# multiplefish/VPLines-SLAM

Hardware: AMD Instinct MI355X
Metric: sliding-window BA solves/sec (10 KF, 200 pts + 80 lines, 5 iters) (higher is better)
Workload: dtype f64

## Files before the change

include/vplines_ba.h:

```cpp
#ifndef VPLINES_BA_H
#define VPLINES_BA_H

#ifdef __cplusplus
extern "C" {
#endif

#define VPL_WINDOW_SIZE 10
#define VPL_NFRAMES 11
#define VPL_MAX_PRIOR_BLOCKS 23
#define VPL_MAX_PRIOR_DIM 171

#define VPL_OK 0
#define VPL_E_INVALID -1
#define VPL_E_NODEVICE -2
#define VPL_E_HIP -3
#define VPL_E_CAPACITY -4
#define VPL_E_NUMERIC -5

#define VPL_MARGIN_OLD 0
#define VPL_MARGIN_SECOND_NEW 1
#define VPL_MARGIN_NONE -1

#define VPL_BLOCK_POSE 0
#define VPL_BLOCK_SPEEDBIAS 1
// ... 266 lines not shown
int vpl_odo_solve_auto(vpl_odo* odo, vpl_odo_result* out);
int vpl_odo_keyframe_auto(vpl_odo* odo, const vpl_odo_frame* next, vpl_odo_result* out);
int vpl_odo_keyframe_imu_auto(vpl_odo* odo, const vpl_odo_imu_frame* next, vpl_odo_result* out, vpl_odo_imu_out* imu_out);

int vpl_odo_get_prior(vpl_odo* odo, int seq, vpl_prior* out);
int vpl_odo_get_states(vpl_odo* odo, int seq, double (*pose)[7], double (*speed_bias)[9], double* ex_pose);
int vpl_odo_get_tracks(vpl_odo* odo, int seq, int* n_points, int* point_id, int* point_start, int* point_nobs, double* inv_depth,
                       int* n_lines, int* line_id, int* line_start, int* line_nobs, int* line_triangulated, double* line_plk);
#define VPL_ODO_D2H_PAD_BYTES 0
int vpl_odo_stats(vpl_odo* odo, long long* h2d_payload_bytes, long long* h2d_table_bytes, long long* d2h_bytes);
int vpl_odo_debug_ms(vpl_odo* odo, double* ms4);

int vpl_odo_debug_tracks(int max_tracks, int n_steps, const int* flag, const int* n_ids, const int* ids, const unsigned char* erase,
                         int* status, int* n_slide, int* slide, int* n_tracks, int* table, int* ignored);
int vpl_odo_debug_parallax_list(int max_tracks, int n_steps, const int* flag, const int* n_ids, const int* ids,
                                const unsigned char* erase, int* n_list, int* list, int* last_track_num);

int vpl_ba_debug_linearization(vpl_ctx* ctx, int window, int* n_points, int* n_lines, int* line_index, double* H, double* g,
                               double* x_pose, double* x_speed_bias, double* x_ex_pose, double* x_inv_depth, double* x_line_orth,
                               double* x_cost);
int vpl_ba_debug_step(vpl_ctx* ctx, int window, double* scale, double* diag, double* grad, double* gn, double* tr14, int* path,
                      double* cand_pose, double* cand_speed_bias, double* cand_ex_pose, double* cand_inv_depth,
                      double* cand_line_orth);

int vpl_ba_enable_kernel_timing(vpl_ctx* ctx, int enable);
int vpl_ba_kernel_times(vpl_ctx* ctx, int* count, const char** names, double* total_ms, int* launches);
int vpl_ba_launch_profile(vpl_ctx* ctx, int* count, const char** names, double* ms, int* active);

int vpl_ba_debug_point_units(int n_points, const int* point_start, const int* point_nobs, int max_rounds,
                             int* lane_table, int* unit_table, int* rounds, int* rounds0);
int vpl_ba_debug_point_chains(const int* unit_table, int rounds, int rounds0, int marg_pass);

#ifdef __cplusplus
}
#endif
#endif
```

vplines-slam_amd/capi.py:

```python
import ctypes as C
import time
import os

import numpy as np

from . import _build

NF = 11
MAX_PRIOR_BLOCKS = 23
MAX_PRIOR_DIM = 171
MARGIN_OLD, MARGIN_SECOND_NEW, MARGIN_NONE = 0, 1, -1
PRIOR_PIVOTED_CHOLESKY, PRIOR_EIGEN = 0, 1
BLOCK_POSE, BLOCK_SPEEDBIAS, BLOCK_EXPOSE = 0, 1, 2

_dp = C.POINTER(C.c_double)
_ip = C.POINTER(C.c_int)


class BaOptions(C.Structure):
    _fields_ = [("num_iterations", C.c_int), ("estimate_extrinsic", C.c_int), ("marginalization_flag", C.c_int),
                ("remove_line_outliers", C.c_int), ("focal_length", C.c_double), ("line_factor", C.c_double),
                ("vp_factor", C.c_double), ("g_norm", C.c_double), ("acc_n", C.c_double), ("gyr_n", C.c_double),
                ("acc_w", C.c_double), ("gyr_w", C.c_double), ("huber_delta", C.c_double)]

# ... 319 lines not shown
    lib.vpl_odo_enable_imu.argtypes = [vp, C.c_int]
    lib.vpl_odo_set_imu.argtypes = [vp, C.c_int, C.c_int, _dp, _dp, _dp]
    lib.vpl_odo_advance_imu.argtypes = [vp, C.POINTER(OdoImuFrame), C.POINTER(OdoResult), C.POINTER(OdoImuOut)]
    lib.vpl_odo_keyframe_imu.argtypes = [vp, C.POINTER(OdoImuFrame), _ip, C.POINTER(OdoResult), C.POINTER(OdoImuOut)]
    lib.vpl_odo_get_preint.argtypes = [vp, C.c_int, C.POINTER(Preintegration)]
    _llp = C.POINTER(C.c_longlong)
    lib.vpl_odo_stats.argtypes = [vp, _llp, _llp, _llp]
    lib.vpl_odo_debug_ms.argtypes = [vp, _dp]
    lib.vpl_odo_debug_tracks.argtypes = [C.c_int, C.c_int, _ip, _ip, _ip, C.POINTER(C.c_ubyte), _ip, _ip, _ip, _ip, _ip, _ip]
    lib.vpl_odo_default_keyframe_rule.argtypes = [C.POINTER(OdoKeyframeRule)]
    lib.vpl_odo_default_keyframe_rule.restype = None
    lib.vpl_odo_enable_keyframe_rule.argtypes = [vp, C.POINTER(OdoKeyframeRule)]
    lib.vpl_odo_get_decision.argtypes = [vp, C.c_int, C.POINTER(OdoDecision)]
    lib.vpl_odo_solve_auto.argtypes = [vp, C.POINTER(OdoResult)]
    lib.vpl_odo_keyframe_auto.argtypes = [vp, C.POINTER(OdoFrame), C.POINTER(OdoResult)]
    lib.vpl_odo_keyframe_imu_auto.argtypes = [vp, C.POINTER(OdoImuFrame), C.POINTER(OdoResult), C.POINTER(OdoImuOut)]
    lib.vpl_failure_default_limits.argtypes = [C.POINTER(FailureLimits)]
    lib.vpl_failure_default_limits.restype = None
    lib.vpl_failure_detection.argtypes = [C.POINTER(FailureLimits), _dp, _dp, _dp]
    lib.vpl_odo_debug_parallax_list.argtypes = [C.c_int, C.c_int, _ip, _ip, _ip, C.POINTER(C.c_ubyte), _ip, _ip, _ip]
    lib.vpl_ba_debug_marg_Ab.argtypes = [vp, C.c_int, _dp, _dp]
    lib.vpl_ba_debug_linearization.argtypes = [vp, C.c_int, _ip, _ip, _ip] + [_dp] * 8
    lib.vpl_ba_debug_step.argtypes = [vp, C.c_int] + [_dp] * 5 + [_ip] + [_dp] * 5
    lib.vpl_ba_debug_allocs.argtypes = [vp, _llp, _llp]
    lib.vpl_ba_debug_psd_factor.argtypes = [vp, C.c_int, C.c_int, C.c_int, _ip, _dp, _dp, _dp, _dp, _ip, _ip, _dp, _dp]
    _hip = lib
    return lib


def _p(a):
    return a.ctypes.data_as(_dp)


class Context:

    def __init__(self, device=0, max_windows=1, max_points=256, max_point_obs=2816, max_lines=128,
                 max_line_obs=1408, stream=None):
        self.lib = load_hip_library()
        self.h = C.c_void_p()
        rc = self.lib.vpl_ctx_create(C.byref(self.h), device, max_windows, max_points, max_point_obs, max_lines,
                                     max_line_obs)
        if rc != 0:
            raise RuntimeError("vpl_ctx_create failed: %d" % rc)
        if stream is not None:
            self.set_stream(stream)
        self._cw = None
# ... 49 lines not shown
                                                 _p(ex), _p(invd), _p(orth), _p(cost))
        if rc != n:
            self._check(rc if rc < 0 else -1, "vpl_ba_debug_linearization")
        return dict(n=n, n_points=nP, n_lines=nL, line_index=idx[:nL].copy(), H=H, g=g, pose=pose, speed_bias=sb, ex_pose=ex,
                    inv_depth=invd[:nP].copy(), line_orth=orth[:nL].copy(), x_cost=float(cost[0]))

    def debug_step(self, w):
        self._settle()
        n, nP, nL = self._debug_counts(w)
        scale, diag, grad, gn = (np.zeros(n) for _ in range(4))
        tr, path = np.zeros(14), C.c_int(-1)
        pose, sb, ex = np.zeros((NF, 7)), np.zeros((NF, 9)), np.zeros(7)
        invd, orth = np.zeros(max(nP, 1)), np.zeros((max(nL, 1), 4))
        rc = self.lib.vpl_ba_debug_step(self.h, w, _p(scale), _p(diag), _p(grad), _p(gn), _p(tr), C.byref(path), _p(pose), _p(sb),
                                        _p(ex), _p(invd), _p(orth))
        if rc != n:
            self._check(rc if rc < 0 else -1, "vpl_ba_debug_step")
        out = dict(n=n, scale=scale, diag=diag, grad=grad, gn=gn, path=path.value, pose_c=pose, speed_bias_c=sb, ex_pose_c=ex,
                   inv_depth_c=invd[:nP].copy(), line_orth_c=orth[:nL].copy())
        for k, f in enumerate(self.TR_FIELDS):
            out[f] = float(tr[k]) if k < 10 else int(tr[k])
        return out

    def close(self):
        if self.h:
            bad = self.debug_guards() if os.environ.get("VPL_DEBUG_GUARDS") == "1" else 0
            msg = self.lib.vpl_last_error(self.h).decode() if bad else ""
            self.lib.vpl_ctx_destroy(self.h)
            self.h = C.c_void_p()
            if bad:
                import sys
                print("vpl_ba_debug_guards: %d arrays overrun; %s" % (bad, msg), file=sys.stderr)
                raise RuntimeError("vpl_ba_debug_guards: %d arrays overrun; %s" % (bad, msg))

    def __del__(self):
        try:
            self.close()
        except Exception:
            pass

    def _check(self, rc, what):
        if rc != 0:
            msg = self.lib.vpl_last_error(self.h)
            raise RuntimeError("%s failed (%d): %s" % (what, rc, msg.decode() if msg else ""))

    def set_stream(self, stream_ptr):
# ... 578 lines not shown
```

vplines-slam_amd/csrc/ba_ctx.h:

```cpp
#pragma once
#include <functional>
#include <map>
#include <string>

#include "vplines_ba.h"
#include "ba_types.h"
#include "ba_stage.h"
#include "ba_restore.h"

struct vpl_ctx {
  int device = 0;
  hipStream_t stream = nullptr;
  DevBatch B;
  std::vector<DevAlloc> allocs;
  bool guards = false;
  std::string err;
  int maxW = 0, maxP = 0, maxPO = 0, maxL = 0, maxLO = 0;
  int nW = 0;
  vpl_ba_options opt;
  bool upload_open = false;
  std::vector<int> h_nP, h_nL;
  std::vector<std::vector<int>> h_lmap;
  std::vector<int> h_mg_m;
  std::vector<int> h_mg_n;
  std::vector<int> h_mg_nb;
  std::vector<int> h_passthrough;
  std::vector<vpl_prior> h_pass_priors;
  bool any_second_new = false;
  int maxPriorN = 0;
  bool prior_resident = false;
  int prior_resident_nW = 0;
  std::vector<int> layout_key;
  bool layout_valid = false;
  bool force_general = false;
  bool schur_mostly_wide = false;
  bool schur_never_wide = false;
  bool schur_wide_all = false;
  bool step_fused = true;
  size_t marg_smem = 0;
  int marg_nmax = 0;
  bool marg_small = false;
  int prior_rule = VPL_PRIOR_PIVOTED_CHOLESKY;
  hipGraphExec_t graph_exec[3] = {nullptr, nullptr, nullptr};
  bool use_graph = true;
  int restore_pending = RESTORE_NONE;
  bool restore_fold = true;
  bool timing = false;
  std::map<std::string, std::pair<double, int>> ktimes;
  std::vector<std::pair<const char*, double>> ltimes;
  int* d_act = nullptr;
  std::vector<std::string> kname_store;
  bool leg_timing = false;
  hipEvent_t leg_ev[6] = {nullptr, nullptr, nullptr, nullptr, nullptr, nullptr};
  double odo_ms[3] = {0, 0, 0};
  std::function<int()> pending;
  Stage stage;
  size_t last_upload_bytes = 0;
  struct vpl_odo* odo = nullptr;
};

static void drop_graph(vpl_ctx* c) {
// ... 71 lines not shown
```

vplines-slam_amd/csrc/ba_lin.h:

```cpp
#pragma once
#include "ba_common.h"

namespace vpl {

typedef double v4d_lin __attribute__((ext_vector_type(4)));
constexpr int LIN_THREADS = 512;
constexpr int STG_LD = 17;
constexpr int LIN_STAGE = 8 * 32 * STG_LD;
constexpr int PRE_LDS = 62;
constexpr int LIN_HW = 720;
constexpr int PREP_NMAX = 112;
__host__ __device__ constexpr int lin_stage_doubles(int maxL) {
  const int ln = 8 * LIN_HW + 38 * maxL;
  const int pt = LIN_STAGE + 78 * 36 + NV;
  const int m = ln > pt ? ln : pt;
  return m > 4650 + 3570 ? m : 4650 + 3570;
}
constexpr int PREP_THREADS = 640;
inline size_t prep_smem(int max_prior_n) {
  const int ns = max_prior_n < PREP_NMAX ? max_prior_n : PREP_NMAX;
  return (size_t)((PREP_THREADS / 64) * 675 + ns * ns + ns + 84) * sizeof(double);
}
constexpr size_t PREP_SMEM = (size_t)((PREP_THREADS / 64) * 675 + PREP_NMAX * PREP_NMAX + PREP_NMAX + 84) * sizeof(double);

__device__ __forceinline__ void prep_body(const DevBatch& B, const int w, double* psm, int nstage, const int restore) {
  const int tid = threadIdx.x;
  const int lane = tid & 63, wv = tid >> 6;
  const int NWV = blockDim.x >> 6;
  double* wsc = psm + wv * 675;
  double* Jl = psm + NWV * 675;
  double* r0s = Jl + nstage * nstage;
  double* xq = r0s + nstage;
  const int nrs = restore ? 99 + B.maxP + (restore > 1 ? 6 * B.maxL : 0) : 0;
  auto rs_src = [&](int i) -> const double* {
    return i < 99 ? B.sb_0 + (size_t)w * 99 + i
                  : i < 99 + B.maxP ? B.invd_0 + (size_t)w * B.maxP + (i - 99) : B.plk_0 + (size_t)w * B.maxL * 6 + (i - 99 - B.maxP);
  };
  auto rs_dst = [&](int i) -> double* {
    return i < 99 ? B.sb + (size_t)w * 99 + i
// ... 723 lines not shown
    const DevPreint& dp = *(const DevPreint*)(plds + PRE_LDS * f);
    bool act = MARG ? (j == 1 && dp.sum_dt < 10.0) : !(dp.sum_dt > 10.0);
    if (PRIOR_ONLY) act = false;
    if (tid < 64) imuact[f] = act ? 1 : 0;
    if (act) {
      PreInt p = load_preint(dp);
      if (tid < 64) {
        imu_residual_raw(p, xp + 7 * (j - 1), xs + 9 * (j - 1), xp + 7 * j, xs + 9 * j, B.opt.g_norm, imur + 15 * f);
      } else {
        ImuJac JB = imu_jacobian_raw(p, xp + 7 * (j - 1), xs + 9 * (j - 1), xp + 7 * j, xs + 9 * j, B.opt.g_norm);
        imu_jac_dense(JB, imuJ + 450 * f);
      }
    }
  }
  __syncthreads();
  VPL_STAMP(B, w, 28);
  constexpr int ASM_PER_THREAD = (NCP + LIN_THREADS - 1) / LIN_THREADS;
  int2 asmd[ASM_PER_THREAD];
#pragma unroll
  for (int u = 0; u < ASM_PER_THREAD; ++u) {
    const int e = u * T + tid;
    asmd[u] = ((const int2*)B.asm_tab)[e < NCP ? e : 0];
  }
  double* imuH = imuJ + 4650;
  {
    const int wvi = tid >> 6, m16 = lane & 15, kk = lane >> 4;
    v4d_lin cd[2] = {{0, 0, 0, 0}, {0, 0, 0, 0}};
    for (int i = tid; i < 120; i += T) imuH[i] = 0.0;
#pragma unroll
    for (int q = 0; q < 2; ++q) {
      const int f = wvi + 8 * q;
      if (f >= 10) break;
      double* J = imuJ + 450 * f;
      double* rr = imur + 15 * f;
      const bool on = imuact[f] != 0;
      v4d_lin jw[2] = {{0, 0, 0, 0}, {0, 0, 0, 0}};
#pragma unroll
      for (int ct = 0; ct < 2; ++ct) {
        const int c = 16 * ct + m16;
#pragma unroll
        for (int ks = 0; ks < 4; ++ks) {
          const int k = 4 * ks + kk;
          const double bv = k < 15 ? (c < 30 ? J[k * 30 + c] : (c == 30 ? rr[k] : 0.0)) : 0.0;
          jw[ct] = __builtin_amdgcn_mfma_f64_16x16x4f64(on ? sa[q][ks] : 0.0, bv, jw[ct], 0, 0, 0);
        }
      }
// ... 67 lines not shown
    for (int k = 0; k < 15; ++k) s += imur[15 * tid + k] * imur[15 * tid + k];
    cost += 0.5 * s;
  }


  if (ROLE == 2) {
    if (tid == 0) {
      while (__hip_atomic_load(&B.lin_flag[w], __ATOMIC_RELAXED, __HIP_MEMORY_SCOPE_AGENT) != 1) __builtin_amdgcn_s_sleep(32);
      __hip_atomic_store(&B.lin_flag[w], 0, __ATOMIC_RELAXED, __HIP_MEMORY_SCOPE_AGENT);
    }
    __syncthreads();
    const double* part = B.lin_part + (size_t)w * LIN_PART;
    for (int i = tid; i < HV_DOUBLES + NV; i += T) sm[i] += __hip_atomic_load(&part[i], __ATOMIC_RELAXED, __HIP_MEMORY_SCOPE_AGENT);
    if (tid == 0) cost += __hip_atomic_load(&part[HV_DOUBLES + NV], __ATOMIC_RELAXED, __HIP_MEMORY_SCOPE_AGENT);
    __syncthreads();
  } else if (!MARG) {
    if (tid == 0) cost += cost_pts;
  }
  VPL_STAMP(B, w, 20);
  double* Hout = B.Hcc + (size_t)w * NCP;
  const double* pH = B.pr_H + (size_t)w * B.prS;
  VPL_STAMP(B, w, 26);
  const bool prior_lds = n > 0 && n <= PRH_N;
  {
#pragma unroll
    for (int u = 0; u < ASM_PER_THREAD; ++u) {
      const int e = u * T + tid;
      if (e >= NCP) continue;
      const int hv = asmd[u].x & 0xffff, im = asmd[u].x >> 16, r = asmd[u].y & 255, c = asmd[u].y >> 8;
      const double vh = Hv[hv ? hv - 1 : 0], vi = imuH[im ? im - 1 : 0];
      const int ir = prior_lds ? invmap[r] : -1, ic = prior_lds ? invmap[c] : -1;
      const bool hp = ir >= 0 && ic >= 0;
      const int hi_ = ic > ir ? ic : ir, lo_ = ic > ir ? ir : ic;
      const double vp = prH[hp ? hi_ * (hi_ + 1) / 2 + lo_ : 0];
      double v = hv ? vh : 0.0;
      v += im ? vi : 0.0;
      v += hp ? vp : 0.0;
      if (!ex_free && r >= 165) v = 0.0;
      Hout[e] = v;
    }
  }
  VPL_STAMP(B, w, 27);
  if (n > PRH_N) {
    __syncthreads();
    const int np = n * (n + 1) / 2;
    for (int base = 0; base < np; base += 4 * T) {
      double ph[4];
      int tr_[4], tc_[4];
#pragma unroll
      for (int u = 0; u < 4; ++u) {
        const int e = base + u * T + tid;
        ph[u] = 0.0; tr_[u] = -1; tc_[u] = 0;
        if (e < np) {
          int i, j;
          tri_decode(e, i, j);
          ph[u] = pH[(size_t)i * n + j];
          const int ri = B.pr_map[(size_t)w * MAXPN + i], rj = B.pr_map[(size_t)w * MAXPN + j];
          tr_[u] = ri > rj ? ri : rj;
          tc_[u] = ri > rj ? rj : ri;
        }
      }
#pragma unroll
      for (int u = 0; u < 4; ++u)
        if (tr_[u] >= 0 && (ex_free || tr_[u] < 165)) Hout[(size_t)tr_[u] * (tr_[u] + 1) / 2 + tc_[u]] += ph[u];
    }
  }
  for (int r = tid; r < NC; r += T) {
    double v = 0.0;
    const int vr = cam2vis(r);
    if (vr >= 0) v += gv[vr];
    if (r < 165) {
      const int fr = r / 15;
      if (fr >= 1 && imuact[fr - 1]) {
        const double* J = imuJ + 450 * (fr - 1);
        const double* rr = imur + 15 * (fr - 1);
        const int a = r - 15 * (fr - 1);
        double s = 0;
#pragma unroll
        for (int k = 0; k < 15; ++k) s += J[k * 30 + a] * rr[k];
        v += s;
      }
      if (fr < 10 && imuact[fr]) {
        const double* J = imuJ + 450 * fr;
        const double* rr = imur + 15 * fr;
        const int a = r - 15 * fr;
        double s = 0;
#pragma unroll
        for (int k = 0; k < 15; ++k) s += J[k * 30 + a] * rr[k];
        v += s;
      }
    }
    if (n > 0 && invmap[r] >= 0) v += prg[invmap[r]];
    if (!ex_free && r >= 165) v = 0.0;
    B.gc[(size_t)w * NC + r] = v;
  }
  VPL_STAMP(B, w, 21);
  cost = block_sum(cost, red);
  if (tid == 0 && !MARG) {
    tr->x_cost = cost;
    if (tr->iter == 0) tr->initial_cost = cost;
    tr->fresh_lin = 1;
    if (tr->iter == 0 && tr->num_successful == 0 && !isfinite(cost)) {
      tr->status = 2; tr->iter = -1; tr->num_successful = -1; tr->x_cost = 0.0; tr->initial_cost = 0.0;
    }
  }
}
template <int MODE>
__global__ __launch_bounds__(LIN_THREADS) void k_lin(DevBatch B) {
  extern __shared__ double sm[];
  lin_body<MODE, 0>(B, MODE == 0 ? ordered_window(B) : (int)blockIdx.x, sm);
}
__global__ __launch_bounds__(LIN_THREADS) void k_lin2(DevBatch B) {
  extern __shared__ double sm[];
  const int nlin = B.ord_it == 0 ? B.nW : B.ord_cnt[2 * (B.ord_it & 1)];
  if (2 * nlin > B.ncu) {
    if ((int)blockIdx.x < B.nW) lin_body<0, 0>(B, ordered_window(B), sm);
    return;
  }
  const int b = (int)(blockIdx.x >> 4) * 8 + (int)(blockIdx.x & 7);
  if (b >= B.nW) return;
// ... 24 lines not shown
```

vplines-slam_amd/csrc/ba_step.h:

```cpp
#pragma once
#include "ba_common.h"
#include "ba_solve.h"

namespace vpl {

constexpr int SCHUR_THREADS = 256;
constexpr int CHOL_THREADS = 256;
constexpr int BACK_THREADS = 256;

__device__ __forceinline__ void lds_ticket_wait(int* t, int seq) {
  while (__hip_atomic_load(t, __ATOMIC_RELAXED, __HIP_MEMORY_SCOPE_WORKGROUP) != seq) __builtin_amdgcn_s_sleep(1);
  __builtin_amdgcn_fence(__ATOMIC_ACQUIRE, "workgroup", "local");
}
__device__ __forceinline__ void lds_ticket_pass(int* t, int seq, int lane) {
  __builtin_amdgcn_fence(__ATOMIC_RELEASE, "workgroup", "local");
  if (lane == 0) __hip_atomic_store(t, seq + 1, __ATOMIC_RELAXED, __HIP_MEMORY_SCOPE_WORKGROUP);
}

__device__ __forceinline__ int compact2vis(int c, int s, int WS) {
  if (c < WS - 6) { const int v = 6 * s + c; return v < 66 ? v : -1; }
  if (c < WS) return 66 + (c - (WS - 6));
  return c < WS + 2 ? 72 + (c - WS) : -1;
}

// ... 128 lines not shown
  double* pS = sm + r1;
  double* pE = pS + B.maxP;
  double* lC = pE + B.maxP;
  double* lS = lC + 10 * B.maxL;
  double* lE = lS + 4 * B.maxL;
  double* lG = lE + 4 * B.maxL;
  double* pG = lG + 4 * B.maxL;
  double* uc = pG + B.maxP;
  double* red = uc + 176;
  int* tick = (int*)(red + 24);
  int* flag = tick + 2;
  int4* etab = (int4*)(((uintptr_t)(flag + 2) + 15) & ~(uintptr_t)15);
  int* ftab = (int*)(etab + B.maxKS);

  {
    const int4* ktab = (const int4*)B.sk_tab + (size_t)w * B.maxKS;
    for (int k = tid; k < B.maxKS; k += T) etab[k] = ktab[k];
  }
  const double* Hcc = B.Hcc + (size_t)w * NCP;
  double* lch = B.lchol + (size_t)w * B.maxL * 10;
  if (tid == 0) { flag[0] = 0; tick[0] = 0; }
  const double mu = tr->mu;
  const bool first = (tr->iter == 0);
  VPL_STAMP(B, w, 0);
  double a1 = 0.0, q = 0.0;
  scale_and_gradient<T, false>(B, w, first, kP, kL, uc, nullptr, nullptr, a1, q);
  __syncthreads();
  double qq = 0.0;
  {
    constexpr int NB = (NZ_N + SCHUR_THREADS - 1) / SCHUR_THREADS;
    constexpr int HALF = (NB + 1) / 2;
#pragma unroll 1
    for (int h0 = 0; h0 < NB; h0 += HALF) {
      int code[HALF];
      double hh[HALF];
#pragma unroll
      for (int u = 0; u < HALF; ++u) {
        const int e = (h0 + u) * T + tid;
        code[u] = (h0 + u < NB && e < NZ_N) ? B.nz_tab[e] : -1;
      }
#pragma unroll
      for (int u = 0; u < HALF; ++u) hh[u] = code[u] >= 0 ? Hcc[code[u] & 0x3fff] : 0.0;
#pragma unroll
      for (int u = 0; u < HALF; ++u)
        if (code[u] >= 0) {
          const int r = (code[u] >> 14) & 255, c = code[u] >> 22;
          qq += (r == c ? 1.0 : 2.0) * uc[r] * hh[u] * uc[c];
        }
    }
  }
  VPL_STAMP(B, w, 1);
  for (int p = tid; p < nP; p += T) {
// ... 210 lines not shown
      flush(gcur, seq);
    }
#ifdef VPL_STAMPS
    if (lane == 0 && wv < 2) {
      long long* dg_ = B.dbg + (size_t)w * 64 + 30 + 6 * wv;
      dg_[0] = st_xf; dg_[1] = st_ld; dg_[2] = st_mf; dg_[3] = st_flush; dg_[4] = st_wait; dg_[5] = nent;
    }
#endif
  }
  __syncthreads();
  VPL_STAMP(B, w, 3);
  for (int b = tid; b < NV; b += T) qq += 2.0 * Cacc[(NV + 1) * CSQ_LD + b] * uc[vis2cam(b)];
  double* sacc = B.sacc + (size_t)w * SACC_N;
  for (int i = tid; i < SACC_N; i += T) {
    int a, b;
    tri_decode(i, a, b);
    sacc[i] = Cacc[a * CSQ_LD + b];
  }
  a1 = block_sum(a1, red);
  q = block_sum(q, red);
  qq = block_sum(qq, red);
  if (tid == 0) {
    tr->a1 = a1;
    tr->alpha = a1 / (q + qq);
    if (flag[0]) B.path[w] = 2;
  }
  VPL_STAMP(B, w, 4);
}

template <int NTC>
__global__ __launch_bounds__(SCHUR_THREADS, 2) void k_schur(DevBatch B) {
  extern __shared__ double sm[];
  empty_next_order(B);
  schur_body<NTC>(B, ordered_window(B), sm);
}
__global__ __launch_bounds__(SCHUR_THREADS, 2) void k_schur_mixed(DevBatch B) {
  extern __shared__ double sm[];
  empty_next_order(B);
  schur_body<3, true>(B, ordered_window(B), sm);
}
inline size_t schur_smem(int maxP, int maxL, int ntc = 5) {
  const int r1 = std::max(4 * maxP + 28 * maxL, (int)CSQ_N);
  const int maxKS = maxP / 4 + maxL + NF + 2;
  return (size_t)(r1 + 3 * maxP + 22 * maxL + 176 + 24) * sizeof(double) + (size_t)(8 + 4 * maxKS + ntc * (ntc + 1) / 2 * 256) * sizeof(int);
}

constexpr int DN = 90;
// ... 388 lines not shown
```

vplines-slam_amd/csrc/ba_trust.h:

```cpp
#pragma once
#include "ba_common.h"

namespace vpl {

constexpr double kMinDiag = 1e-6, kMaxDiag = 1e32, kMaxMu = 1.0, kMuIncrease = 10.0;
constexpr double kMinRelDecrease = 1e-3, kFuncTol = 1e-6, kParamTol = 1e-8, kMinRadius = 1e-32;
constexpr int kMaxInvalid = 5;

__device__ __forceinline__ void chol4(double* A, bool& ok) {
#pragma unroll
  for (int j = 0; j < 4; ++j) {
    double d = A[tri(j, j)];
#pragma unroll
    for (int k = 0; k < 4; ++k) if (k < j) d -= A[tri(j, k)] * A[tri(j, k)];
    if (!(d > 0.0)) { ok = false; d = 1.0; }
    d = sqrt(d);
    A[tri(j, j)] = d;
#pragma unroll
    for (int i = 0; i < 4; ++i) if (i > j) {
      double s2 = A[tri(i, j)];
#pragma unroll
      for (int k = 0; k < 4; ++k) if (k < j) s2 -= A[tri(i, k)] * A[tri(j, k)];
      A[tri(i, j)] = s2 / d;
    }
  }
}

__device__ __forceinline__ void empty_next_order(const DevBatch& B) {
  if (blockIdx.x == 0 && threadIdx.x == 0) { B.ord_cnt[2 * ((B.ord_it + 1) & 1)] = 0; B.ord_cnt[2 * ((B.ord_it + 1) & 1) + 1] = 0; }
}

template <int T, bool KEEP>
__device__ __forceinline__ void scale_and_gradient(const DevBatch& B, const int w, const bool first, double* kP, double* kL, double* uc,
                                                   double* sc, double* dg, double& a1, double& q) {
  const int tid = threadIdx.x;
  const int nP = B.nP[w], nL = B.nL[w];
  const size_t fb = (size_t)w * B.nfull;
  double* gscale = B.scale + fb;
  double* gdiag = B.diag + fb;
  double* ggrad = B.grad + fb;
  const double* Hcc = B.Hcc + (size_t)w * NCP;
  const double* gc = B.gc + (size_t)w * NC;
  const int LP = NC, LL = NC + B.maxP;
  double pre_hp = 0.0, pre_sp = 0.0, pre_gp = 0.0, pre_Hl[16], pre_sl[4], pre_gl[4];
  if (tid < nP) {
    const size_t pi = (size_t)w * B.maxP + tid;
    pre_hp = B.Hpp[pi]; pre_gp = B.gp[pi];
    if (!first) pre_sp = gscale[LP + tid];
  }
#pragma unroll
  for (int k = 0; k < 16; ++k) pre_Hl[k] = 0.0;
#pragma unroll
  for (int a = 0; a < 4; ++a) { pre_sl[a] = 0.0; pre_gl[a] = 0.0; }
  if (tid < nL) {
    const size_t li = (size_t)w * B.maxL + tid;
#pragma unroll
    for (int k = 0; k < 16; ++k) pre_Hl[k] = B.Hll[li * 16 + k];
#pragma unroll
    for (int a = 0; a < 4; ++a) {
      pre_gl[a] = B.gl[li * 4 + a];
      if (!first) pre_sl[a] = gscale[LL + 4 * tid + a];
    }
  }
  for (int c = tid; c < 176; c += T) {
    double s = 0.0, d = 1.0, g = 0.0;
    if (c < NC) {
      const double h = Hcc[tri(c, c)];
      s = first ? 1.0 / (1.0 + sqrt(h)) : gscale[c];
      if (first) gscale[c] = s;
      d = sqrt(fmin(fmax(s * s * h, kMinDiag), kMaxDiag));
      g = s * gc[c] / d;
      gdiag[c] = d; ggrad[c] = g;
      a1 += g * g;
    }
    if constexpr (KEEP) { sc[c] = s; dg[c] = d; }
    uc[c] = s * g / d;
  }
  for (int p = tid; p < nP; p += T) {
    const size_t pi = (size_t)w * B.maxP + p;
    const bool pre = p == tid;
    const double h = pre ? pre_hp : B.Hpp[pi];
    const double s = first ? 1.0 / (1.0 + sqrt(h)) : (pre ? pre_sp : gscale[LP + p]);
    if (first) gscale[LP + p] = s;
    const double d = sqrt(fmin(fmax(s * s * h, kMinDiag), kMaxDiag));
    const double g = s * (pre ? pre_gp : B.gp[pi]) / d;
    gdiag[LP + p] = d; ggrad[LP + p] = g;
    kP[4 * p] = s; kP[4 * p + 1] = d; kP[4 * p + 2] = g; kP[4 * p + 3] = h;
    a1 += g * g;
    const double u = s * g / d;
    q += u * h * u;
  }
  for (int l = tid; l < nL; l += T) {
    const size_t li = (size_t)w * B.maxL + l;
    const bool pre = l == tid;
    double Hl[16], sl4[4], gl4[4];
#pragma unroll
    for (int k = 0; k < 16; ++k) Hl[k] = pre ? pre_Hl[k] : B.Hll[li * 16 + k];
#pragma unroll
    for (int a = 0; a < 4; ++a) {
// ... 303 lines not shown
```

vplines-slam_amd/csrc/ba_types.h:

```cpp
#pragma once
#include <stdint.h>

namespace vpl {

constexpr int NF = 11;
constexpr int NC = 171;
constexpr int NV = 72;
__host__ __device__ inline int wcol(int c, int s, int WS) {
  if (c >= 66) return WS - 72 + c;
  const int cc = c - 6 * s;
  return (cc >= 0 && cc < WS - 6) ? cc : -1;
}
constexpr int NCP = NC * (NC + 1) / 2;
constexpr int MAXPB = 23;
constexpr int MAXPN = 171;
constexpr int ACT_SLOTS = 64;
constexpr int SK_WSTRIDE = 64;
constexpr int NZ_N = 2628 + 1089 + 1890 + 540;
constexpr int SACC_N = 74 * 75 / 2;
constexpr int MAXKEEP = 80;

__host__ __device__ inline int vis2cam(int v) { return v < 66 ? 15 * (v / 6) + (v % 6) : 165 + (v - 66); }
__host__ __device__ inline int tri(int r, int c) { return r * (r + 1) / 2 + c; }

// ... 62 lines not shown
  int *pr_kind, *pr_frame, *pr_idx;
  double *pr_x0;
  double *pr_J0, *pr_r0;
  double *pr_H;
  double *pr_g0;
  int prS;
  int *pr_map;

  double *Hcc, *gc;
  int *asm_tab;
  double *Hpp, *gp, *Wp;
  double *Hll, *gl, *Wl;
  int WS, wfill;
  int *order;
  int *ord_cnt;
  int ord_it;
  double *lchol;

  int *sk_tab, *sk_wave;
  int maxKS;
  double *sacc;
  double *ycs;
  double *sx;
  int *path;
  int step_fused;
  int *nz_tab;

  TrState *tr;
  double *scale, *diag, *grad, *gn;

  int *mg_n, *mg_nb;
  int *mg_kind, *mg_frame, *mg_idx, *mg_cam;
  double *mg_x0;
  double *mg_J0, *mg_r0;
  double *mg_A, *mg_b;
  int *mg_m;
  long long *dbg;
  int *act;
  int launch;
};


struct KeepSrc {
  int nP; const int *pt_start, *pt_nobs;
  int nL; const int *ln_start, *ln_nobs, *ln_removed;
  int pr_nb; const int *pr_kind, *pr_frame;
  bool imu01;
};
// ... 53 lines not shown
```

vplines-slam_amd/csrc/vplines_ba.hip:

```cpp
#include <hip/hip_runtime.h>

#include <algorithm>
#include <chrono>
#include <memory>
#include <cstdlib>
#include <cstring>
#include <string>
#include <vector>

#include "vplines_ba.h"
#include "ba_types.h"
#include "ba_lin.h"
#include "ba_pack.h"
#include "ba_solve.h"
#include "ba_step.h"
#include "ba_marg.h"
#include "ba_prior_eig.h"
#include "ba_lineopt.h"
#include "ba_factors.h"
#include "ba_odo.h"
#include "odo_tracks.h"
#include "host_common.h"

using namespace vpl;
// ... 95 lines not shown
  AL(pose_c, W * 77); AL(sb_c, W * 99); AL(ex_c, W * 7); AL(invd_c, W * B.maxP); AL(orth_c, W * B.maxL * 4); AL(lw, W * B.maxL * 6); AL(lw_c, W * B.maxL * 6);
  AL(lin_part, W * LIN_PART); AL(lin_pcost, W); AL(lin_flag, W);
  AL(pose_0, W * 77); AL(sb_0, W * 99); AL(ex_0, W * 7); AL(invd_0, W * B.maxP); AL(plk_0, W * B.maxL * 6);
  AL(plk, W * B.maxL * 6); AL(gauge, W * 4); AL(fail_ref, W * 13); AL(orth_in, W);
  AL(nP, W); AL(nL, W);
  AL(pt_start, W * B.maxP); AL(pt_nobs, W * B.maxP); AL(pt_off, W * B.maxP); AL(pt_obs, W * B.maxPO * 3);
  AL(ps_list, W * B.maxP); AL(ps_cnt, W * (NF + 1)); AL(pu_lane, W * B.maxPR * 1024); AL(pu_sub, W * B.maxPR * 512); AL(pu_cnt, W); AL(pu_cnt0, W);
  AL(ln_start, W * B.maxL); AL(ln_nobs, W * B.maxL); AL(ln_off, W * B.maxL); AL(ln_obs, W * B.maxLO * 8);
  AL(nLO, W); AL(lo_ln, W * B.maxLO);
  AL(ll_tab, W * B.llSlots * 2); AL(ll_np, W);
  AL(pre, W * NF);
  AL(pr_n, W); AL(pr_nb, W); AL(pr_kind, W * MAXPB); AL(pr_frame, W * MAXPB); AL(pr_idx, W * MAXPB);
  AL(pr_x0, W * MAXPB * 9); AL(pr_J0, W * MAXPN * MAXPN); AL(pr_r0, W * MAXPN); AL(pr_H, W * MAXPN * MAXPN); AL(pr_g0, W * MAXPN);
  AL(pr_map, W * MAXPN);
  AL(Hcc, W * NCP); AL(gc, W * NC); AL(asm_tab, 2 * NCP); AL(Hpp, W * B.maxP); AL(gp, W * B.maxP); AL(Wp, W * B.maxP * NV);
  AL(Hll, W * B.maxL * 16); AL(gl, W * B.maxL * 4); AL(Wl, W * B.maxL * 4 * NV); AL(lchol, W * B.maxL * 10);
  AL(tr, W);
  AL(scale, W * B.nfull); AL(diag, W * B.nfull); AL(grad, W * B.nfull); AL(gn, W * B.nfull);
  AL(mg_n, W); AL(mg_nb, W); AL(mg_kind, W * MAXPB); AL(mg_frame, W * MAXPB); AL(mg_idx, W * MAXPB);
  AL(mg_cam, W * MAXPB); AL(mg_x0, W * MAXPB * 9); AL(mg_J0, W * MAXKEEP * MAXKEEP); AL(mg_r0, W * MAXKEEP);
  AL(mg_A, W * MAXKEEP * MAXKEEP); AL(mg_b, W * MAXKEEP); AL(mg_m, W); AL(dbg, W * 64); AL(ln_removed, W * B.maxL); AL(ln_tri, W * B.maxL);
  if (e == hipSuccess) e = dalloc(c, &c->d_act, (size_t)ACT_SLOTS * 4);
  AL(order, 2 * W); AL(ord_cnt, 4);
  AL(sk_tab, W * B.maxKS * 4); AL(sk_wave, W * 8 * SK_WSTRIDE); AL(sacc, W * SACC_N); AL(nz_tab, NZ_N); AL(ycs, W * 176); AL(sx, W * 8); AL(path, W);
#undef AL
  if (e != hipSuccess) return VPL_E_HIP;
  if (lin_smem_base(c->maxP, c->maxL) > LIN_LDS_BUDGET) return VPL_E_CAPACITY;
  B.prhN = lin_prh_n(c->maxP, c->maxL);
  {
    std::vector<int> tab(2 * NCP);
    for (int r = 0, e2 = 0; r < NC; ++r)
      for (int cc = 0; cc <= r; ++cc, ++e2) lin_asm_entry(r, cc, &tab[2 * e2]);
    if (hipMemcpy(B.asm_tab, tab.data(), tab.size() * sizeof(int), hipMemcpyHostToDevice) != hipSuccess) return VPL_E_HIP;
  }
  {
    std::vector<int> nz;
    for (int r = 0; r < NC; ++r)
      for (int cc = 0; cc <= r; ++cc) {
        const bool vis = cam2vis(r) >= 0 && cam2vis(cc) >= 0;
        const int fr = r < 165 ? r / 15 : -1, fc = cc < 165 ? cc / 15 : -1;
        const bool band = fr >= 0 && fc >= 0 && (fr == fc || fr == fc + 1);
        const bool sb0 = cc >= 6 && cc < 15 && cam2vis(r) >= 0;
        if (vis || band || sb0) nz.push_back(tri(r, cc) | r << 14 | cc << 22);
      }
    if ((int)nz.size() != NZ_N || hipMemcpy(B.nz_tab, nz.data(), nz.size() * sizeof(int), hipMemcpyHostToDevice) != hipSuccess) return VPL_E_HIP;
  }
  static size_t lin_max = 0, solve_max = 0, schur_max = 0, back_max = 0, step_max = 0;
  lin_max = std::max(lin_max, lin_smem(c->maxP, c->maxL));
  solve_max = std::max(solve_max, solve_smem(c->maxP, c->maxL));
  schur_max = std::max(schur_max, schur_smem(c->maxP, c->maxL));
  back_max = std::max(back_max, back_smem(c->maxP, c->maxL));
  step_max = std::max(step_max, step_smem(c->maxP, c->maxL));
  if (schur_max > 159 * 1024 || back_max > 159 * 1024) return VPL_E_CAPACITY;
  const std::pair<const void*, size_t> lds[] = {
      {(const void*)k_lin2, lin_max}, {(const void*)k_lin<1>, lin_max}, {(const void*)k_lin<2>, lin_max},
      {(const void*)k_solve, solve_max}, {(const void*)k_schur<3>, schur_max}, {(const void*)k_schur<5>, schur_max},
      {(const void*)k_schur_mixed, schur_max}, {(const void*)k_chol, CHOL_SMEM}, {(const void*)k_back, back_max},
      {(const void*)k_step<3, false>, step_max}, {(const void*)k_step<3, true>, step_max}, {(const void*)k_step<5, false>, step_max},
      {(const void*)k_prep, PREP_SMEM}, {(const void*)k_marg<MARG_THREADS>, 159 * 1024}, {(const void*)k_marg<256>, MARG_LDS_SMALL},
      {(const void*)k_prior_eigen, prior_eig_layout(MAXKEEP).bytes}, {(const void*)k_init_align, init_lds_bytes(INIT_NMAX)}};
  for (const auto& k : lds)
    if (hipFuncSetAttribute(k.first, hipFuncAttributeMaxDynamicSharedMemorySize, (int)k.second) != hipSuccess) return VPL_E_HIP;
  vpl_ba_default_options(&c->opt);
  if (const char* gv = std::getenv("VPL_BA_GRAPH")) c->use_graph = std::atoi(gv) != 0;
  if (const char* gv = std::getenv("VPL_BA_GENERAL")) c->force_general = std::atoi(gv) != 0;
  if (const char* gv = std::getenv("VPL_BA_STEP_FUSED")) c->step_fused = std::atoi(gv) != 0;
  if (const char* gv = std::getenv("VPL_BA_RESET_FOLD")) c->restore_fold = std::atoi(gv) != 0;
  if (const char* gv = std::getenv("VPL_BA_SCHUR_WIDE")) { c->schur_wide_all = std::atoi(gv) > 0; c->schur_never_wide = std::atoi(gv) < 0; }
  return VPL_OK;
}

int vpl_ctx_create(vpl_ctx** out, int device, int max_windows, int max_points, int max_point_obs, int max_lines,
                   int max_line_obs) {
  if (!out || max_windows < 1 || max_points < 0 || max_lines < 0) return VPL_E_INVALID;
  int ndev = 0;
  if (hipGetDeviceCount(&ndev) != hipSuccess || ndev == 0 || device >= ndev) return VPL_E_NODEVICE;
  if (hipSetDevice(device) != hipSuccess) return VPL_E_NODEVICE;
  vpl_ctx* c = new vpl_ctx();
  const int rc = ctx_init(c, device, max_windows, max_points, max_point_obs, max_lines, max_line_obs);
  if (rc != VPL_OK) {
    free_arrays(c);
    delete c;
    return rc;
  }
  *out = c;
  return VPL_OK;
}

void vpl_ctx_destroy(vpl_ctx* c) {
  if (!c) return;
// ... 403 lines not shown
    for (size_t w = 0; w < W; ++w) {
      vpl_window& v = win[w];
      if (reports) std::memset(&reports[w], 0, sizeof(reports[w]));
      if (c->h_lmap[w].size() < 4) {
        if (v.line_removed) std::fill(v.line_removed, v.line_removed + v.n_lines, 0);
        continue;
      }
      const int nrem = scatter_solved_lines(c, w, v, &(*plk)[w * maxL * 6], &(*removed)[w * maxL]);
      if (reports) {
        fill_report(reports[w], (*tr)[w]);
        reports[w].n_lines_removed = nrem;
      }
    }
    return VPL_OK;
  });
}
int vpl_ba_only_line_opt(vpl_ctx* c, int nW, vpl_window* win, const vpl_ba_options* opt, vpl_solve_report* reports) {
  return only_line_opt_impl(c, nW, win, opt, reports, false);
}
int vpl_ba_only_line_opt_async(vpl_ctx* c, int nW, vpl_window* win, const vpl_ba_options* opt, vpl_solve_report* reports) {
  return only_line_opt_impl(c, nW, win, opt, reports, true);
}

static void launch_solve(vpl_ctx* c, int w0, int nw, hipStream_t s, int restore) {
  DevBatch B = c->B;
  B.ord_it = 0;
  B.act = c->timing ? c->d_act : nullptr;
  B.launch = 0;
  B.step_fused = c->step_fused && !c->timing;
  if (c->timing) { c->ltimes.clear(); (void)hipMemsetAsync(c->d_act, 0, sizeof(int) * ACT_SLOTS * 4, s); }
  const dim3 grid(nw);
  launch_prep(c, B, nw, s, restore);
  ++B.launch;
  { KTimer t(c, "k_lin"); hipLaunchKernelGGL(k_lin2, dim3(16 * ((nw + 7) / 8)), dim3(LIN_THREADS), lin_smem(c->maxP, c->maxL), s, B); }
  ++B.launch;
  const bool narrow = B.WS + 2 <= 48, wide = !narrow && (c->schur_wide_all || (c->schur_mostly_wide && !c->schur_never_wide));
  const int ntc = wide ? 5 : 3;
  void (*const kstep)(DevBatch) = narrow ? k_step<3, false> : wide ? k_step<5, false> : k_step<3, true>;
  void (*const kschur)(DevBatch) = narrow ? k_schur<3> : wide ? k_schur<5> : k_schur_mixed;
  for (int it = 0; it < c->opt.num_iterations; ++it) {
    B.ord_it = it;
    if (B.step_fused) {
      hipLaunchKernelGGL(kstep, grid, dim3(SCHUR_THREADS), step_smem(B.maxP, B.maxL, ntc), s, B);
      ++B.launch;
      hipLaunchKernelGGL(k_solve, grid, dim3(SOLVE_THREADS), solve_smem(B.maxP, B.maxL), s, B);
      ++B.launch;
    } else {
      { KTimer t(c, "k_schur"); hipLaunchKernelGGL(kschur, grid, dim3(SCHUR_THREADS), schur_smem(B.maxP, B.maxL, ntc), s, B); }
      ++B.launch;
      { KTimer t(c, "k_chol"); hipLaunchKernelGGL(k_chol, grid, dim3(CHOL_THREADS), CHOL_SMEM, s, B); }
      ++B.launch;
      { KTimer t(c, "k_solve"); hipLaunchKernelGGL(k_solve, grid, dim3(SOLVE_THREADS), solve_smem(B.maxP, B.maxL), s, B); }
// ... 399 lines not shown
  const int rc = debug_window_ready(c, w);
  if (rc) return rc;
  const DevBatch& B = c->B;
  const int nP = c->h_nP[w], nL = (int)c->h_lmap[w].size();
  if (nP < 0 || nP > B.maxP || nL > B.maxL) return fail(c, VPL_E_INVALID, "debug read-out: counts outside the context's capacity");
  int rs = debug_full_vector(c, w, nP, nL, B.scale, scale);
  if (!rs) rs = debug_full_vector(c, w, nP, nL, B.diag, diag);
  if (!rs) rs = debug_full_vector(c, w, nP, nL, B.grad, grad);
  if (!rs) rs = debug_full_vector(c, w, nP, nL, B.gn, gn);
  if (rs) return rs;
  if (tr14) {
    TrState t;
    HIPCHK(c, hipMemcpy(&t, B.tr + w, sizeof(t), hipMemcpyDeviceToHost));
    const double v[14] = {t.radius, t.mu, t.alpha, t.a1, t.a2, t.a3, t.model_cost_change, t.dogleg_step_norm, t.step_norm, t.x_norm,
                          (double)t.iter, (double)t.status, (double)t.num_successful, (double)t.step_valid};
    std::memcpy(tr14, v, sizeof(v));
  }
  if (path) HIPCHK(c, hipMemcpy(path, B.path + w, 4, hipMemcpyDeviceToHost));
  rs = debug_states(c, w, nP, nL, B.pose_c, B.sb_c, B.ex_c, B.invd_c, B.orth_c, cand_pose, cand_speed_bias, cand_ex_pose,
                    cand_inv_depth, cand_line_orth);
  return rs ? rs : NC + nP + 4 * nL;
}

int vpl_ba_debug_psd_factor(vpl_ctx* c, int form, int threads, int n_cases, const int* n, const double* A, const double* b,
                            const double* abs_tol, const double* rel_tol, int* rank, int* perm, double* J0, double* r0) {
  if (!c || n_cases < 1 || !n || !A || !b || !abs_tol || !rel_tol || !rank || !perm || !J0 || !r0) return VPL_E_INVALID;
  const int nlim = form == 0 ? 16 : form == 1 ? 48 : form == 2 ? 76 : form == 3 ? MAXKEEP : 0;
  const bool pairing = (form == 0 && threads == 256) || (form == 2 && threads == 512) ||
                       ((form == 1 || form == 3) && (threads == 256 || threads == 512));
  if (!pairing) return fail(c, VPL_E_INVALID, "debug_psd_factor: this form does not run on this many threads");
  int nmax = 0;
  for (int i = 0; i < n_cases; ++i) {
    if (n[i] < 1 || n[i] > nlim) return fail(c, VPL_E_INVALID, "debug_psd_factor: n outside the form's range");
    nmax = std::max(nmax, n[i]);
  }
  HIPCHK(c, hipSetDevice(c->device));
  const size_t N = (size_t)n_cases, M2 = (size_t)MAXKEEP * MAXKEEP;
  DevBuf dn, dA, db, dat, drt, drank, dperm, dJ, dr;
  HIPCHK(c, dn.alloc(N * 4)); HIPCHK(c, dA.alloc(N * M2 * 8)); HIPCHK(c, db.alloc(N * MAXKEEP * 8));
  HIPCHK(c, dat.alloc(N * 8)); HIPCHK(c, drt.alloc(N * 8)); HIPCHK(c, drank.alloc(N * 4)); HIPCHK(c, dperm.alloc(N * MAXKEEP * 4));
  HIPCHK(c, dJ.alloc(N * M2 * 8)); HIPCHK(c, dr.alloc(N * MAXKEEP * 8));
  HIPCHK(c, hipMemcpyAsync(dn.p, n, N * 4, hipMemcpyHostToDevice, c->stream));
  HIPCHK(c, hipMemcpyAsync(dA.p, A, N * M2 * 8, hipMemcpyHostToDevice, c->stream));
  HIPCHK(c, hipMemcpyAsync(db.p, b, N * MAXKEEP * 8, hipMemcpyHostToDevice, c->stream));
  HIPCHK(c, hipMemcpyAsync(dat.p, abs_tol, N * 8, hipMemcpyHostToDevice, c->stream));
  HIPCHK(c, hipMemcpyAsync(drt.p, rel_tol, N * 8, hipMemcpyHostToDevice, c->stream));
// ... 94 lines not shown
```

Baseline: 266,300.

## Fold camera-block Cauchy quadratic term into linearization assembly

Moves the camera gradient assembly ahead of the Hessian assembly in the linearization kernel. While the camera Hessian is being written, it also accumulates u^T H_cc u, where u is the scaled gradient direction, and stores the result per window. The step kernel then skips its own pass over the nonzero camera Hessian table and adds the stored value into the Cauchy alpha denominator. In exchange the linearization kernel gains a block sync, extra LDS and a reduction, and the fold only applies when the prior Hessian fits in LDS.

```diff
diff --git a/include/vplines_ba.h b/include/vplines_ba.h
--- a/include/vplines_ba.h
+++ b/include/vplines_ba.h
@@ -312,6 +312,7 @@
 int vpl_ba_debug_step(vpl_ctx* ctx, int window, double* scale, double* diag, double* grad, double* gn, double* tr14, int* path,
                       double* cand_pose, double* cand_speed_bias, double* cand_ex_pose, double* cand_inv_depth,
                       double* cand_line_orth);
+int vpl_ba_debug_cauchy_cam(vpl_ctx* ctx, int window, double* cq);
 
 int vpl_ba_enable_kernel_timing(vpl_ctx* ctx, int enable);
 int vpl_ba_kernel_times(vpl_ctx* ctx, int* count, const char** names, double* total_ms, int* launches);
diff --git a/vplines-slam_amd/capi.py b/vplines-slam_amd/capi.py
--- a/vplines-slam_amd/capi.py
+++ b/vplines-slam_amd/capi.py
@@ -365,6 +365,7 @@
     lib.vpl_ba_debug_marg_Ab.argtypes = [vp, C.c_int, _dp, _dp]
     lib.vpl_ba_debug_linearization.argtypes = [vp, C.c_int, _ip, _ip, _ip] + [_dp] * 8
     lib.vpl_ba_debug_step.argtypes = [vp, C.c_int] + [_dp] * 5 + [_ip] + [_dp] * 5
+    lib.vpl_ba_debug_cauchy_cam.argtypes = [vp, C.c_int, _dp]
     lib.vpl_ba_debug_allocs.argtypes = [vp, _llp, _llp]
     lib.vpl_ba_debug_psd_factor.argtypes = [vp, C.c_int, C.c_int, C.c_int, _ip, _dp, _dp, _dp, _dp, _ip, _ip, _dp, _dp]
     _hip = lib
@@ -460,6 +461,14 @@
             out[f] = float(tr[k]) if k < 10 else int(tr[k])
         return out
 
+    def debug_cauchy_cam(self, w):
+        self._settle()
+        cq = np.zeros(1)
+        rc = self.lib.vpl_ba_debug_cauchy_cam(self.h, w, _p(cq))
+        if rc < 0:
+            self._check(rc, "vpl_ba_debug_cauchy_cam")
+        return float(cq[0]) if rc == 1 else None
+
     def close(self):
         if self.h:
             bad = self.debug_guards() if os.environ.get("VPL_DEBUG_GUARDS") == "1" else 0
diff --git a/vplines-slam_amd/csrc/ba_ctx.h b/vplines-slam_amd/csrc/ba_ctx.h
--- a/vplines-slam_amd/csrc/ba_ctx.h
+++ b/vplines-slam_amd/csrc/ba_ctx.h
@@ -37,6 +37,7 @@
   bool schur_never_wide = false;
   bool schur_wide_all = false;
   bool step_fused = true;
+  bool cauchy_fold = true;
   size_t marg_smem = 0;
   int marg_nmax = 0;
   bool marg_small = false;
diff --git a/vplines-slam_amd/csrc/ba_lin.h b/vplines-slam_amd/csrc/ba_lin.h
--- a/vplines-slam_amd/csrc/ba_lin.h
+++ b/vplines-slam_amd/csrc/ba_lin.h
@@ -1,5 +1,6 @@
 #pragma once
 #include "ba_common.h"
+#include "ba_trust.h"
 
 namespace vpl {
 
@@ -14,7 +15,7 @@
   const int ln = 8 * LIN_HW + 38 * maxL;
   const int pt = LIN_STAGE + 78 * 36 + NV;
   const int m = ln > pt ? ln : pt;
-  return m > 4650 + 3570 ? m : 4650 + 3570;
+  return m > 4650 + 3570 + 176 ? m : 4650 + 3570 + 176;
 }
 constexpr int PREP_THREADS = 640;
 inline size_t prep_smem(int max_prior_n) {
@@ -784,6 +785,10 @@
     const int e = u * T + tid;
     asmd[u] = ((const int2*)B.asm_tab)[e < NCP ? e : 0];
   }
+  const bool cq_on = !MARG && B.cauchy_fold != 0;
+  const bool cq_first = tr->iter == 0;
+  double cq_scale = 0.0;
+  if (cq_on && !cq_first && tid < NC) cq_scale = B.scale[(size_t)w * B.nfull + tid];
   double* imuH = imuJ + 4650;
   {
     const int wvi = tid >> 6, m16 = lane & 15, kk = lane >> 4;
@@ -897,6 +902,54 @@
   const double* pH = B.pr_H + (size_t)w * B.prS;
   VPL_STAMP(B, w, 26);
   const bool prior_lds = n > 0 && n <= PRH_N;
+  double* ucq = imuH + 3570;
+  for (int r = tid; r < NC; r += T) {
+    double v = 0.0, u = 0.0;
+    const int vr = cam2vis(r);
+    if (vr >= 0) v += gv[vr];
+    if (r < 165) {
+      const int fr = r / 15;
+      if (fr >= 1 && imuact[fr - 1]) {
+        const double* J = imuJ + 450 * (fr - 1);
+        const double* rr = imur + 15 * (fr - 1);
+        const int a = r - 15 * (fr - 1);
+        double s = 0;
+#pragma unroll
+        for (int k = 0; k < 15; ++k) s += J[k * 30 + a] * rr[k];
+        v += s;
+      }
+      if (fr < 10 && imuact[fr]) {
+        const double* J = imuJ + 450 * fr;
+        const double* rr = imur + 15 * fr;
+        const int a = r - 15 * fr;
+        double s = 0;
+#pragma unroll
+        for (int k = 0; k < 15; ++k) s += J[k * 30 + a] * rr[k];
+        v += s;
+      }
+    }
+    if (n > 0 && invmap[r] >= 0) v += prg[invmap[r]];
+    if (!ex_free && r >= 165) v = 0.0;
+    B.gc[(size_t)w * NC + r] = v;
+    if (cq_on) {
+      const int hv = vr >= 0 ? hvi(vr, vr) + 1 : 0;
+      const int ar = r - 15 * (r / 15);
+      const int im = r < 165 ? 120 * (r / 15) + ar * (ar + 1) / 2 + ar + 1 : 0;
+      const double vh = Hv[hv ? hv - 1 : 0], vi = imuH[im ? im - 1 : 0];
+      const int ir = prior_lds ? invmap[r] : -1;
+      const double vp = prH[ir >= 0 ? ir * (ir + 1) / 2 + ir : 0];
+      double h = hv ? vh : 0.0;
+      h += im ? vi : 0.0;
+      h += ir >= 0 ? vp : 0.0;
+      if (!ex_free && r >= 165) h = 0.0;
+      double s, d, g;
+      cam_scale_diag_u(h, v, cq_first, cq_scale, s, d, g, u);
+      ucq[r] = u;
+    }
+  }
+  if (cq_on && tid >= NC && tid < 176) ucq[tid] = 0.0;
+  double cqs = 0.0;
+  if (cq_on) __syncthreads();
   {
 #pragma unroll
     for (int u = 0; u < ASM_PER_THREAD; ++u) {
@@ -913,6 +966,7 @@
       v += hp ? vp : 0.0;
       if (!ex_free && r >= 165) v = 0.0;
       Hout[e] = v;
+      if (cq_on) cqs += (r == c ? 1.0 : 2.0) * ucq[r] * v * ucq[c];
     }
   }
   VPL_STAMP(B, w, 27);
@@ -940,37 +994,12 @@
         if (tr_[u] >= 0 && (ex_free || tr_[u] < 165)) Hout[(size_t)tr_[u] * (tr_[u] + 1) / 2 + tc_[u]] += ph[u];
     }
   }
-  for (int r = tid; r < NC; r += T) {
-    double v = 0.0;
-    const int vr = cam2vis(r);
-    if (vr >= 0) v += gv[vr];
-    if (r < 165) {
-      const int fr = r / 15;
-      if (fr >= 1 && imuact[fr - 1]) {
-        const double* J = imuJ + 450 * (fr - 1);
-        const double* rr = imur + 15 * (fr - 1);
-        const int a = r - 15 * (fr - 1);
-        double s = 0;
-#pragma unroll
-        for (int k = 0; k < 15; ++k) s += J[k * 30 + a] * rr[k];
-        v += s;
-      }
-      if (fr < 10 && imuact[fr]) {
-        const double* J = imuJ + 450 * fr;
-        const double* rr = imur + 15 * fr;
-        const int a = r - 15 * fr;
-        double s = 0;
-#pragma unroll
-        for (int k = 0; k < 15; ++k) s += J[k * 30 + a] * rr[k];
-        v += s;
-      }
-    }
-    if (n > 0 && invmap[r] >= 0) v += prg[invmap[r]];
-    if (!ex_free && r >= 165) v = 0.0;
-    B.gc[(size_t)w * NC + r] = v;
-  }
   VPL_STAMP(B, w, 21);
   cost = block_sum(cost, red);
+  if (cq_on) {
+    cqs = block_sum(cqs, red);
+    if (tid == 0) B.cq[w] = cqs;
+  }
   if (tid == 0 && !MARG) {
     tr->x_cost = cost;
     if (tr->iter == 0) tr->initial_cost = cost;
diff --git a/vplines-slam_amd/csrc/ba_step.h b/vplines-slam_amd/csrc/ba_step.h
--- a/vplines-slam_amd/csrc/ba_step.h
+++ b/vplines-slam_amd/csrc/ba_step.h
@@ -174,12 +174,13 @@
   if (tid == 0) { flag[0] = 0; tick[0] = 0; }
   const double mu = tr->mu;
   const bool first = (tr->iter == 0);
+  const double cqw = B.cauchy_fold ? B.cq[w] : 0.0;
   VPL_STAMP(B, w, 0);
   double a1 = 0.0, q = 0.0;
   scale_and_gradient<T, false>(B, w, first, kP, kL, uc, nullptr, nullptr, a1, q);
   __syncthreads();
   double qq = 0.0;
-  {
+  if (!B.cauchy_fold) {
     constexpr int NB = (NZ_N + SCHUR_THREADS - 1) / SCHUR_THREADS;
     constexpr int HALF = (NB + 1) / 2;
 #pragma unroll 1
@@ -436,7 +437,7 @@
   qq = block_sum(qq, red);
   if (tid == 0) {
     tr->a1 = a1;
-    tr->alpha = a1 / (q + qq);
+    tr->alpha = a1 / (q + (qq + cqw));
     if (flag[0]) B.path[w] = 2;
   }
   VPL_STAMP(B, w, 4);
diff --git a/vplines-slam_amd/csrc/ba_trust.h b/vplines-slam_amd/csrc/ba_trust.h
--- a/vplines-slam_amd/csrc/ba_trust.h
+++ b/vplines-slam_amd/csrc/ba_trust.h
@@ -28,6 +28,14 @@
 
 __device__ __forceinline__ void empty_next_order(const DevBatch& B) {
   if (blockIdx.x == 0 && threadIdx.x == 0) { B.ord_cnt[2 * ((B.ord_it + 1) & 1)] = 0; B.ord_cnt[2 * ((B.ord_it + 1) & 1) + 1] = 0; }
+}
+
+__device__ __forceinline__ void cam_scale_diag_u(const double h, const double gcv, const bool first, const double stored, double& s,
+                                                 double& d, double& g, double& u) {
+  s = first ? 1.0 / (1.0 + sqrt(h)) : stored;
+  d = sqrt(fmin(fmax(s * s * h, kMinDiag), kMaxDiag));
+  g = s * gcv / d;
+  u = s * g / d;
 }
 
 template <int T, bool KEEP>
@@ -63,18 +71,16 @@
     }
   }
   for (int c = tid; c < 176; c += T) {
-    double s = 0.0, d = 1.0, g = 0.0;
+    double s = 0.0, d = 1.0, g = 0.0, u = 0.0;
     if (c < NC) {
       const double h = Hcc[tri(c, c)];
-      s = first ? 1.0 / (1.0 + sqrt(h)) : gscale[c];
+      cam_scale_diag_u(h, gc[c], first, first ? 0.0 : gscale[c], s, d, g, u);
       if (first) gscale[c] = s;
-      d = sqrt(fmin(fmax(s * s * h, kMinDiag), kMaxDiag));
-      g = s * gc[c] / d;
       gdiag[c] = d; ggrad[c] = g;
       a1 += g * g;
     }
     if constexpr (KEEP) { sc[c] = s; dg[c] = d; }
-    uc[c] = s * g / d;
+    uc[c] = u;
   }
   for (int p = tid; p < nP; p += T) {
     const size_t pi = (size_t)w * B.maxP + p;
diff --git a/vplines-slam_amd/csrc/ba_types.h b/vplines-slam_amd/csrc/ba_types.h
--- a/vplines-slam_amd/csrc/ba_types.h
+++ b/vplines-slam_amd/csrc/ba_types.h
@@ -108,8 +108,10 @@
   double *sacc;
   double *ycs;
   double *sx;
+  double *cq;
   int *path;
   int step_fused;
+  int cauchy_fold;
   int *nz_tab;
 
   TrState *tr;
diff --git a/vplines-slam_amd/csrc/vplines_ba.hip b/vplines-slam_amd/csrc/vplines_ba.hip
--- a/vplines-slam_amd/csrc/vplines_ba.hip
+++ b/vplines-slam_amd/csrc/vplines_ba.hip
@@ -141,7 +141,7 @@
   AL(mg_A, W * MAXKEEP * MAXKEEP); AL(mg_b, W * MAXKEEP); AL(mg_m, W); AL(dbg, W * 64); AL(ln_removed, W * B.maxL); AL(ln_tri, W * B.maxL);
   if (e == hipSuccess) e = dalloc(c, &c->d_act, (size_t)ACT_SLOTS * 4);
   AL(order, 2 * W); AL(ord_cnt, 4);
-  AL(sk_tab, W * B.maxKS * 4); AL(sk_wave, W * 8 * SK_WSTRIDE); AL(sacc, W * SACC_N); AL(nz_tab, NZ_N); AL(ycs, W * 176); AL(sx, W * 8); AL(path, W);
+  AL(sk_tab, W * B.maxKS * 4); AL(sk_wave, W * 8 * SK_WSTRIDE); AL(sacc, W * SACC_N); AL(nz_tab, NZ_N); AL(ycs, W * 176); AL(sx, W * 8); AL(path, W); AL(cq, W);
 #undef AL
   if (e != hipSuccess) return VPL_E_HIP;
   if (lin_smem_base(c->maxP, c->maxL) > LIN_LDS_BUDGET) return VPL_E_CAPACITY;
@@ -185,6 +185,7 @@
   if (const char* gv = std::getenv("VPL_BA_GENERAL")) c->force_general = std::atoi(gv) != 0;
   if (const char* gv = std::getenv("VPL_BA_STEP_FUSED")) c->step_fused = std::atoi(gv) != 0;
   if (const char* gv = std::getenv("VPL_BA_RESET_FOLD")) c->restore_fold = std::atoi(gv) != 0;
+  if (const char* gv = std::getenv("VPL_BA_CAUCHY_FOLD")) c->cauchy_fold = std::atoi(gv) != 0;
   if (const char* gv = std::getenv("VPL_BA_SCHUR_WIDE")) { c->schur_wide_all = std::atoi(gv) > 0; c->schur_never_wide = std::atoi(gv) < 0; }
   return VPL_OK;
 }
@@ -634,12 +635,15 @@
   return only_line_opt_impl(c, nW, win, opt, reports, true);
 }
 
+static bool cauchy_folded(const vpl_ctx* c) { return c->cauchy_fold && c->maxPriorN <= c->B.prhN; }
+
 static void launch_solve(vpl_ctx* c, int w0, int nw, hipStream_t s, int restore) {
   DevBatch B = c->B;
   B.ord_it = 0;
   B.act = c->timing ? c->d_act : nullptr;
   B.launch = 0;
   B.step_fused = c->step_fused && !c->timing;
+  B.cauchy_fold = cauchy_folded(c);
   if (c->timing) { c->ltimes.clear(); (void)hipMemsetAsync(c->d_act, 0, sizeof(int) * ACT_SLOTS * 4, s); }
   const dim3 grid(nw);
   launch_prep(c, B, nw, s, restore);
@@ -1085,6 +1089,14 @@
   return rs ? rs : NC + nP + 4 * nL;
 }
 
+int vpl_ba_debug_cauchy_cam(vpl_ctx* c, int w, double* cq) {
+  const int rc = debug_window_ready(c, w);
+  if (rc) return rc;
+  if (!cauchy_folded(c)) return 0;
+  if (cq) HIPCHK(c, hipMemcpy(cq, c->B.cq + w, 8, hipMemcpyDeviceToHost));
+  return 1;
+}
+
 int vpl_ba_debug_psd_factor(vpl_ctx* c, int form, int threads, int n_cases, const int* n, const double* A, const double* b,
                             const double* abs_tol, const double* rel_tol, int* rank, int* perm, double* J0, double* r0) {
   if (!c || n_cases < 1 || !n || !A || !b || !abs_tol || !rel_tol || !rank || !perm || !J0 || !r0) return VPL_E_INVALID;
```

Measured after the change: 265,700. About the same (-0.2%).
